# microscopy-processing/FlowDenoising

Hardware: NVIDIA B200
Metric: Mvoxels/s OF-Gaussian denoise (higher is better)
Workload: dtype f32

## Files before the change

### flowdenoising_b200/csrc/flow.cu

```cuda
#include <math.h>
#include <stdlib.h>
#include <string.h>

#include <atomic>

#include "fdn_internal.cuh"

namespace fdn {

struct FlowIterArgs {
    const float* R;
    int64_t R_stride;
    SlotMap map0, map1;
    const float* flow_in;
    float* flow_out;
    int h, w, m;
    int n;
    int LS;
    int strips;
    double scale;
    double* carry;
    unsigned long long* flags;
    unsigned long long epoch;
    unsigned* ctl;
// ... 160 lines not shown
        constexpr bool kStatic = MT > 0 && TR == 2 * MT + 2;
        const bool steady = kStatic && y0 >= TR && y0 + TR - 1 + m <= h - 1 && y0 + m >= 5 && y0 + TR - 1 + m < h - 5;
        if (active && steady) {
            if constexpr (kStatic) {
                constexpr int RRs = 2 * MT + 2;
                double* tq = tile + q;
                float* rg = ring + t;
#pragma unroll
                for (int r = 0; r < TR; r++) {
                    update_matrices_px<false>(R0a, R0b, R1a, R1b, fl[r], xcl, y0 + r + MT, h, w, Mv, colb, sxc);
#pragma unroll
                    for (int c = 0; c < 5; c++) {
                        rg[(((MT + r) % RRs) * 5 + c) * NT] = Mv[c];
                        const float d = __fsub_rn(Mv[c], rg[(((MT + 1 + r) % RRs) * 5 + c) * NT]);
                        vs[c] = __dadd_rn(vs[c], (double)d);
                        tq[(r * 5 + c) * LS] = vs[c];
                    }
                }
                next_row += TR;
            }
        } else if (active) {
            double* tq = tile + q;
#pragma unroll
            for (int r = 0; r < TR; r++) {
                const int y = y0 + r;
                if (y < h) {
                    if (next_row <= min(y + m, h - 1)) {
                        update_matrices_px(R0a, R0b, R1a, R1b, fl[r], xcl, next_row, h, w, Mv);
#pragma unroll
                        for (int c = 0; c < 5; c++) ring_new[c * NT] = Mv[c];
                        ring_new += 5 * NT;
                        if (ring_new >= ring_end) ring_new -= RR * 5 * NT;
                        next_row++;
                    } else {
                        const float* last = (ring_new == ring + t ? ring_end + t : ring_new) - 5 * NT;
#pragma unroll
                        for (int c = 0; c < 5; c++) Mv[c] = last[c * NT];
                    }
#pragma unroll
                    for (int c = 0; c < 5; c++) {
                        const float d = __fsub_rn(Mv[c], ring_old[c * NT]);
                        vs[c] = __dadd_rn(vs[c], (double)d);
                        tq[(r * 5 + c) * LS] = vs[c];
                    }
                    if (y >= m + 1) {
                        ring_old += 5 * NT;
                        if (ring_old >= ring_end) ring_old -= RR * 5 * NT;
                    }
                }
            }
        }
        if (t == 0 && k > 0) {
            const unsigned long long want = a.epoch + (unsigned long long)tile_idx + 1ull;
            while (*flag_in < want) __nanosleep(20);
            __threadfence();
        }
        __syncthreads();
        if (active) {
#pragma unroll
            for (int r = 0; r < TR; r++) {
                const int row = y0 + TR + r + m;
                if (row < h) fl[r] = __ldg(fin + row * w + xcl);
            }
        }
        if (t < 5 * TR) {
            const int r = t / 5, c = t - r * 5;
            const int y = y0 + r;
            if (y < h) {
                double* line = tile + (r * 5 + c) * LS;
                double S;
                if (k == 0) {
                    S = __dmul_rn(line[m + 1], (double)(m + 2));
                    for (int x = 1; x < m; x++) S = __dadd_rn(S, line[m + 1 + x]);
                } else {
                    S = __ldcg(carry_in + (int64_t)y * 5 + c);
                }
                const int off = 2 * m + 1;
                constexpr int HB = 8;
                int i = 0;
                if (ncols >= HB) {
                    double d[HB];
#pragma unroll
                    for (int u = 0; u < HB; u++) d[u] = __dsub_rn(line[u + off], line[u]);
                    for (; i + 2 * HB <= ncols; i += HB) {
                        double d2[HB];
#pragma unroll
                        for (int u = 0; u < HB; u++) d2[u] = __dsub_rn(line[i + HB + u + off], line[i + HB + u]);
#pragma unroll
                        for (int u = 0; u < HB; u++) {
                            S = __dadd_rn(S, d[u]);
                            line[i + u] = S;
                        }
#pragma unroll
                        for (int u = 0; u < HB; u++) d[u] = d2[u];
                    }
#pragma unroll
                    for (int u = 0; u < HB; u++) {
                        S = __dadd_rn(S, d[u]);
                        line[i + u] = S;
                    }
                    i += HB;
                }
                for (; i < ncols; i++) {
                    S = __dadd_rn(S, __dsub_rn(line[i + off], line[i]));
                    line[i] = S;
                }
                if (k + 1 < a.strips) {
                    __stcg(carry_out + (int64_t)y * 5 + c, S);
                    __threadfence();
                }
            }
        }
        __syncthreads();
        if (t == 0 && k + 1 < a.strips) *flag_out = a.epoch + (unsigned long long)tile_idx + 1ull;
        if (core) {
            const double* tt = tile + t;
#pragma unroll
            for (int r = 0; r < TR; r++) {
                const int y = y0 + r;
                if (y < h) {
                    double g[5];
#pragma unroll
                    for (int c = 0; c < 5; c++) g[c] = __dmul_rn(tt[(r * 5 + c) * LS], a.scale);
                    const double det = __dadd_rn(__dsub_rn(__dmul_rn(g[0], g[2]), __dmul_rn(g[1], g[1])), 1e-3);
                    const double idet = __drcp_rn(det);
                    float2 o;
                    o.x = (float)__dmul_rn(__dsub_rn(__dmul_rn(g[0], g[4]), __dmul_rn(g[1], g[3])), idet);
                    o.y = (float)__dmul_rn(__dsub_rn(__dmul_rn(g[2], g[3]), __dmul_rn(g[1], g[4])), idet);
                    fout[y * w + x0 + t] = o;
                }
            }
        }
        __syncthreads();
    }
    if (t == 0) {
        __threadfence();
        if (atomicAdd(a.ctl + 1, 1u) == gridDim.x - 1) { a.ctl[0] = 0; a.ctl[1] = 0; }
    }
}


struct RowIn {
    float2 f;
    float4 c03;
    float c4;
};

template <int MT, int NT_>
struct WsCfg {
    static constexpr int NT = NT_;
    static constexpr int RR = 2 * MT + 2;
    static constexpr int TR = 5 * RR <= 32 ? RR : RR / 2;
    static constexpr int TPP = RR / TR;
#ifndef FDN_WS_SR4
#define FDN_WS_SR4 2
#endif
    static constexpr int SR = MT == 4 ? FDN_WS_SR4 : 3;
    static constexpr int NB = (TR + SR - 1) / SR;
    static constexpr int HALO = 2 * MT + 1;
    static constexpr int CWMAX = (NT - HALO) & ~3;
    static constexpr int NCH = (CWMAX + 31) / 32;
    static constexpr int LS = NT + 2;
#ifndef FDN_WS_NBUF
#define FDN_WS_NBUF 2
#endif
    static constexpr int NBUF = FDN_WS_NBUF;
    static constexpr size_t tiles_bytes = NBUF * sizeof(double) * TR * 5 * LS + 128;
    static constexpr size_t smem_bytes = tiles_bytes + 8 * NBUF * NCH + 16;
    static_assert(5 * TR <= 32, "phase H runs in one warp");
    static_assert(TR * TPP == RR && (TPP == 1 || TPP == 2), "a ring period is one tile or the two shared-memory tiles");
    static_assert(HALO + 8 <= 17, "the scan's register window spans two 8-column sets and one more column");
};

struct Taps {
    float4 p00, p01, p10, p11;
    float q00, q01, q10, q11;
};

template <int PF>
__device__ __forceinline__ Taps ws_gather(const float2 f, const float4* __restrict__ R1a, const float* __restrict__ R1b,
                                          int x, int y, int h, int w)
{
    const int x1 = (int)floorf(__fadd_rn((float)x, f.x)), y1 = (int)floorf(__fadd_rn((float)y, f.y));
    const int yc = min(max(y1, 0), h - 2), xc = min(max(x1, 0), w - 2);
    const int g = yc * w + xc;
    if (PF > 0) {
        const int gp = min(yc + PF + 1, h - 1) * w + xc;
        asm volatile("prefetch.global.L1 [%0];" :: "l"(R1a + gp));
        asm volatile("prefetch.global.L1 [%0];" :: "l"(R1b + gp));
    }
    Taps t;
    t.p00 = __ldg(R1a + g); t.p01 = __ldg(R1a + g + 1); t.p10 = __ldg(R1a + g + w); t.p11 = __ldg(R1a + g + w + 1);
    t.q00 = __ldg(R1b + g); t.q01 = __ldg(R1b + g + 1); t.q10 = __ldg(R1b + g + w); t.q11 = __ldg(R1b + g + w + 1);
    return t;
}

__device__ __forceinline__ void ws_matrices_px(const RowIn& in, const Taps& tp, int x, int y, int h, int w, float sxc,
                                               float M[5])
{
    const float dx = in.f.x, dy = in.f.y;
    float fx = __fadd_rn((float)x, dx), fy = __fadd_rn((float)y, dy);
    const int x1 = (int)floorf(fx), y1 = (int)floorf(fy);
    fx = __fsub_rn(fx, (float)x1);
    fy = __fsub_rn(fy, (float)y1);
    const float4 c03 = in.c03;
    const float c4 = in.c4;
    const bool in_img = (unsigned)x1 < (unsigned)(w - 1) && (unsigned)y1 < (unsigned)(h - 1);
    const float ofx = __fsub_rn(1.f, fx), ofy = __fsub_rn(1.f, fy);
    const float a00 = __fmul_rn(ofx, ofy), a01 = __fmul_rn(fx, ofy), a10 = __fmul_rn(ofx, fy), a11 = __fmul_rn(fx, fy);
#define FDN_BILIN(v00, v01, v10, v11) \
    __fadd_rn(__fadd_rn(__fadd_rn(__fmul_rn(a00, v00), __fmul_rn(a01, v01)), __fmul_rn(a10, v10)), __fmul_rn(a11, v11))
    float r2 = FDN_BILIN(tp.p00.x, tp.p01.x, tp.p10.x, tp.p11.x);
    float r3 = FDN_BILIN(tp.p00.y, tp.p01.y, tp.p10.y, tp.p11.y);
    float r4 = FDN_BILIN(tp.p00.z, tp.p01.z, tp.p10.z, tp.p11.z);
    float r5 = FDN_BILIN(tp.p00.w, tp.p01.w, tp.p10.w, tp.p11.w);
    float r6 = FDN_BILIN(tp.q00, tp.q01, tp.q10, tp.q11);
#undef FDN_BILIN
    r4 = __fmul_rn(__fadd_rn(c03.z, r4), 0.5f);
    r5 = __fmul_rn(__fadd_rn(c03.w, r5), 0.5f);
    r6 = __fmul_rn(__fadd_rn(c4, r6), 0.25f);
    r2 = in_img ? r2 : 0.f;
    r3 = in_img ? r3 : 0.f;
    r4 = in_img ? r4 : c03.z;
    r5 = in_img ? r5 : c03.w;
    r6 = in_img ? r6 : __fmul_rn(c4, 0.5f);
    r2 = __fmul_rn(__fsub_rn(c03.x, r2), 0.5f);
    r3 = __fmul_rn(__fsub_rn(c03.y, r3), 0.5f);
    r2 = __fadd_rn(r2, __fadd_rn(__fmul_rn(r4, dy), __fmul_rn(r6, dx)));
    r3 = __fadd_rn(r3, __fadd_rn(__fmul_rn(r6, dy), __fmul_rn(r5, dx)));
    float s = sxc;
    s = __fmul_rn(s, y < 5 ? (y < 2 ? 0.14f : 0.4472f) : 1.f);
    s = __fmul_rn(s, y >= h - 5 ? (h - y - 1 < 2 ? 0.14f : 0.4472f) : 1.f);
    r2 = __fmul_rn(r2, s); r3 = __fmul_rn(r3, s); r4 = __fmul_rn(r4, s);
    r5 = __fmul_rn(r5, s); r6 = __fmul_rn(r6, s);
    M[0] = __fadd_rn(__fmul_rn(r4, r4), __fmul_rn(r6, r6));
    M[1] = __fmul_rn(__fadd_rn(r4, r5), r6);
    M[2] = __fadd_rn(__fmul_rn(r5, r5), __fmul_rn(r6, r6));
    M[3] = __fadd_rn(__fmul_rn(r4, r2), __fmul_rn(r6, r3));
    M[4] = __fadd_rn(__fmul_rn(r6, r2), __fmul_rn(r5, r3));
}

__device__ __forceinline__ double ws_win(const double2 (&W0)[4], const double2 (&W1)[4], const double2& X, int idx)
{
    return idx < 8 ? ((idx & 1) ? W0[idx >> 1].y : W0[idx >> 1].x)
                   : idx < 16 ? ((idx & 1) ? W1[(idx - 8) >> 1].y : W1[(idx - 8) >> 1].x) : X.x;
}
template <int OFF>
__device__ __forceinline__ void ws_diffs(double (&D)[8], const double2 (&W0)[4], const double2 (&W1)[4], const double2& X)
{
#pragma unroll
    for (int u = 0; u < 8; u++) D[u] = __dsub_rn(ws_win(W0, W1, X, u + OFF), ws_win(W0, W1, X, u));
}

#ifdef FDN_WS_EXPERIMENTS
#define FDN_WS_EXP(bit) (wa.exp & (bit))
#else
#define FDN_WS_EXP(bit) (0)
#endif
#ifndef FDN_WS_HC
#define FDN_WS_HC 8
#endif
#ifndef FDN_WS_PF
#define FDN_WS_PF 6
#endif
#ifndef FDN_WS_L2PF
#define FDN_WS_L2PF 0
#endif
#ifndef FDN_WS_SOLVE_SLEEP
#define FDN_WS_SOLVE_SLEEP 100
#endif
#define FDN_WS_MAX_ITERS 3

struct WsArgs {
    const float* R;
    int64_t R_stride;
    SlotMap map0, map1;
    const float* fin[FDN_WS_MAX_ITERS];
    float* fout[FDN_WS_MAX_ITERS];
    int n, iters;
    int h, w, CW, strips;
    double scale;
    int exp;
    unsigned tag;
    ulonglong2* packets;
    unsigned* ctl;
    unsigned* done;
};

__device__ __forceinline__ void nbar_sync(int id, int count)
{
    asm volatile("bar.sync %0, %1;" :: "r"(id), "r"(count) : "memory");
}
__device__ __forceinline__ void nbar_arrive(int id, int count)
{
    asm volatile("bar.arrive %0, %1;" :: "r"(id), "r"(count) : "memory");
}
__device__ __forceinline__ unsigned ld_acquire_u32(const unsigned* p)
{
    unsigned v;
    asm volatile("ld.acquire.gpu.global.u32 %0, [%1];" : "=r"(v) : "l"(p) : "memory");
    return v;
}

template <int MT, int NT_>
__global__ void __launch_bounds__(NT_ + 128, 2)
k_flow_iter_ws(WsArgs wa)
{
    using C = WsCfg<MT, NT_>;
    constexpr int NT = C::NT, TR = C::TR, SR = C::SR, RR = C::RR, TPP = C::TPP, NB = C::NB, LS = C::LS, NCH = C::NCH, m = MT;
    constexpr int NBUF = C::NBUF, BAR_FULL = 1, BAR_FREE = 1 + NBUF, BAR_SOLVED = 1 + 2 * NBUF;
    constexpr unsigned WARPS = (NT + 128) / 32;
    extern __shared__ __align__(128) unsigned char smem_ws[];
    double* tiles = reinterpret_cast<double*>(smem_ws);
    unsigned long long* chunk_bar = reinterpret_cast<unsigned long long*>(smem_ws + C::tiles_bytes);
    volatile int* sh = reinterpret_cast<volatile int*>(smem_ws + C::tiles_bytes + 8 * NBUF * NCH);
    const int h = wa.h, w = wa.w;
    const int t = threadIdx.x;
    const unsigned per_it = (unsigned)wa.n * (unsigned)wa.strips;
    if (t == 0) {
        const unsigned tk = atomicAdd(wa.ctl, 1u);
        sh[0] = (int)tk;
        const unsigned it0 = tk / per_it;
        if (it0 > 0) {
            const unsigned b0 = (tk - it0 * per_it) / (unsigned)wa.strips;
            const unsigned* dn = wa.done + (size_t)(it0 - 1) * wa.n + b0;
            while (ld_acquire_u32(dn) < (unsigned)wa.strips) __nanosleep(200);
        }
    }
    if (t < NBUF * NCH) mbar_init(smem_u32(chunk_bar + t), 1);
    __syncthreads();
    const unsigned ticket = (unsigned)sh[0];
    const int it = (int)(ticket / per_it);
    const unsigned rem = ticket - (unsigned)it * per_it;
    const int b = (int)(rem / (unsigned)wa.strips);
    const int k = (int)(rem - (unsigned)b * wa.strips);
    const unsigned tag = wa.tag + (unsigned)it;
    const int CW = wa.CW;
    const int x0 = k * CW;
    const int ncols = min(CW, w - x0);
    const int ntiles = (h + TR - 1) / TR;

    auto warp_exit = [&]() {
        __syncwarp();
        unsigned last = 0;
        if ((t & 31) == 0) {
            __threadfence();
            last = atomicAdd(wa.ctl + 1, 1u) == gridDim.x * WARPS - 1u;
        }
        last = __shfl_sync(0xffffffffu, last, 0);
        if (last) {
            for (int i = t & 31; i < wa.iters * wa.n; i += 32) wa.done[i] = 0;
            if ((t & 31) == 0) { wa.ctl[0] = 0; wa.ctl[1] = 0; }
        }
    };

    if (t >= NT) {
#ifndef FDN_WS_RC4
#define FDN_WS_RC4 168
#define FDN_WS_RS4 88
#endif
        if (MT == 4) asm volatile("setmaxnreg.dec.sync.aligned.u32 %0;" :: "n"(FDN_WS_RS4));
        else asm volatile("setmaxnreg.dec.sync.aligned.u32 80;");
        if (t >= NT + 32) {
            constexpr int NS = 96;
            const int sl = t - (NT + 32);
            float2* fout = reinterpret_cast<float2*>(wa.fout[it]) + (int64_t)b * h * w;
            auto solve_px = [&](const double* tt, int r, float2* dst) {
                double g[5];
#pragma unroll
                for (int c = 0; c < 5; c++) g[c] = __dmul_rn(tt[(r * 5 + c) * LS], wa.scale);
                const double det = __dadd_rn(__dsub_rn(__dmul_rn(g[0], g[2]), __dmul_rn(g[1], g[1])), 1e-3);
                const double idet = __drcp_rn(det);
                float2 o;
                o.x = (float)__dmul_rn(__dsub_rn(__dmul_rn(g[0], g[4]), __dmul_rn(g[1], g[3])), idet);
                o.y = (float)__dmul_rn(__dsub_rn(__dmul_rn(g[2], g[3]), __dmul_rn(g[1], g[4])), idet);
                *dst = o;
            };
            const int sw = sl >> 5, sln = sl & 31;
            const int qlast = (ncols - 1) >> 5;
            for (int j = 0; j < ntiles; j++) {
                const int y0 = j * TR;
                const int buf = j % NBUF;
                const uint32_t bars = smem_u32(chunk_bar + buf * NCH);
                const uint32_t parity = (uint32_t)((j / NBUF) & 1);
                for (int q = sw; q <= qlast; q += NS / 32) {
                    mbar_wait_sleep<FDN_WS_SOLVE_SLEEP>(bars + 8 * q, parity);
                    const int col = q * 32 + sln;
                    if (col < ncols && !FDN_WS_EXP(8)) {
                        const double* tt = tiles + buf * TR * 5 * LS + col;
                        float2* dst = fout + (int64_t)y0 * w + x0 + col;
                        if (y0 + TR <= h) {
#pragma unroll
                            for (int r = 0; r < TR; r++) solve_px(tt, r, dst + r * w);
                        } else {
                            for (int r = 0; r < h - y0; r++) solve_px(tt, r, dst + r * w);
                        }
                    }
                }
                mbar_wait_sleep<FDN_WS_SOLVE_SLEEP>(bars + 8 * qlast, parity);
                nbar_arrive(BAR_FREE + buf, NS + NT);
            }
            if (it + 1 < wa.iters) {
                nbar_sync(BAR_SOLVED, NS);
                if (sl == 0) {
                    __threadfence();
                    atomicAdd(wa.done + (size_t)it * wa.n + b, 1u);
                }
            }
            warp_exit();
            return;
        }
        const int lane = t - NT;
        const int r = lane / 5, c = lane - r * 5;
        ulonglong2* pk_out = wa.packets + ((int64_t)b * wa.strips + k) * h * 5;
        const ulonglong2* pk_in = wa.packets + ((int64_t)b * wa.strips + max(k - 1, 0)) * h * 5;
        constexpr int off = 2 * m + 1;
        static_assert(FDN_WS_HC == 8, "the sliding window below is written for 8-column chunks");
        for (int j = 0; j < ntiles; j++) {
            const int y = j * TR + r;
            const int buf = j % NBUF;
            const uint32_t bars = smem_u32(chunk_bar + buf * NCH);
            nbar_sync(BAR_FULL + buf, NT + 32);
            const unsigned hmask = __ballot_sync(0xffffffffu, lane < 5 * TR && y < h);
            if (lane < 5 * TR && y < h) {
                double* line = tiles + (buf * TR * 5 + r * 5 + c) * LS;
                double2* l2 = reinterpret_cast<double2*>(line);
#define FDN_LOADSET(W, kk)                                                        \
    { W[0] = l2[4 * (kk)]; W[1] = l2[4 * (kk) + 1]; W[2] = l2[4 * (kk) + 2]; W[3] = l2[4 * (kk) + 3];   \
      if (off > 7) xx_ = l2[4 * (kk) + 4]; }
#define FDN_CHAIN8(D, kk)                                                          \
    {                                                                              \
        double2 s0, s1, s2, s3;                                                    \
        S = __dadd_rn(S, D[0]); s0.x = S; S = __dadd_rn(S, D[1]); s0.y = S;        \
        S = __dadd_rn(S, D[2]); s1.x = S; S = __dadd_rn(S, D[3]); s1.y = S;        \
        S = __dadd_rn(S, D[4]); s2.x = S; S = __dadd_rn(S, D[5]); s2.y = S;        \
        S = __dadd_rn(S, D[6]); s3.x = S; S = __dadd_rn(S, D[7]); s3.y = S;        \
        l2[4 * (kk)] = s0; l2[4 * (kk) + 1] = s1; l2[4 * (kk) + 2] = s2; l2[4 * (kk) + 3] = s3; \
    }
#define FDN_CHUNK_DONE(kk)                                                         \
    if (((kk) & 3) == 0 && 8 * (kk) < ncols) {                                     \
        __syncwarp(hmask);                                                         \
        if (lane == 0) mbar_arrive(bars + 8 * (((kk) >> 2) - 1));                  \
    }
                const int n8 = ncols >> 3;
                double2 wa_[4], wb_[4], xx_ = make_double2(0., 0.);
                double d[8];
                FDN_LOADSET(wa_, 0);
                FDN_LOADSET(wb_, 1);
                double S;
                if (k == 0) {
                    S = __dmul_rn(line[m + 1], (double)(m + 2));
#pragma unroll
                    for (int x = 1; x < m; x++) S = __dadd_rn(S, line[m + 1 + x]);
                } else if (FDN_WS_EXP(2)) {
                    S = 0.;
                } else {
                    const ulonglong2* src = pk_in + (int64_t)y * 5 + c;
                    ulonglong2 v = __ldcv(src);
                    while ((unsigned)(v.x >> 32) != tag || (unsigned)(v.y >> 32) != tag) {
                        __nanosleep(32);
                        v = __ldcv(src);
                    }
                    S = __hiloint2double((int)(unsigned)v.y, (int)(unsigned)v.x);
                }
                __syncwarp(hmask);
                if (!FDN_WS_EXP(1)) {
                    ws_diffs<off>(d, wa_, wb_, xx_);
                    int kk = 0;
                    while (kk < n8) {
                        FDN_LOADSET(wa_, kk + 2);
                        FDN_CHAIN8(d, kk);
                        ws_diffs<off>(d, wb_, wa_, xx_);
                        ++kk;
                        FDN_CHUNK_DONE(kk);
                        if (kk == n8) break;
                        FDN_LOADSET(wb_, kk + 2);
                        FDN_CHAIN8(d, kk);
                        ws_diffs<off>(d, wa_, wb_, xx_);
                        ++kk;
                        FDN_CHUNK_DONE(kk);
                    }
                    if (ncols & 4) {
                        double2 s0, s1;
                        S = __dadd_rn(S, d[0]); s0.x = S; S = __dadd_rn(S, d[1]); s0.y = S;
                        S = __dadd_rn(S, d[2]); s1.x = S; S = __dadd_rn(S, d[3]); s1.y = S;
                        l2[4 * n8] = s0; l2[4 * n8 + 1] = s1;
                    }
                }
#undef FDN_LOADSET
#undef FDN_CHAIN8
#undef FDN_CHUNK_DONE
                if (k + 1 < wa.strips) {
                    ulonglong2 o;
                    const unsigned long long tg = (unsigned long long)tag << 32;
                    o.x = tg | (unsigned)__double2loint(S);
                    o.y = tg | (unsigned)__double2hiint(S);
                    __stcg(pk_out + (int64_t)y * 5 + c, o);
                }
            }
            __syncwarp();
            if (lane == 0) mbar_arrive(bars + 8 * ((ncols - 1) >> 5));
        }
        warp_exit();
        return;
    }

    if (MT == 4) asm volatile("setmaxnreg.inc.sync.aligned.u32 %0;" :: "n"(FDN_WS_RC4));
    else asm volatile("setmaxnreg.inc.sync.aligned.u32 176;");
    const int xcl = min(max(x0 - m - 1 + t, 0), w - 1);
    const float sxc = __fmul_rn(xcl < 5 ? (xcl < 2 ? 0.14f : 0.4472f) : 1.f,
                                xcl >= w - 5 ? (w - xcl - 1 < 2 ? 0.14f : 0.4472f) : 1.f);

    const float* R0 = wa.R + (int64_t)wa.map0.slot(b) * wa.R_stride;
    const float* R1 = wa.R + (int64_t)wa.map1.slot(b) * wa.R_stride;
    const float4* R0a = reinterpret_cast<const float4*>(R0);
    const float* R0b = R0 + (int64_t)4 * h * w;
    const float4* R1a = reinterpret_cast<const float4*>(R1);
    const float* R1b = R1 + (int64_t)4 * h * w;
    const float2* fin = reinterpret_cast<const float2*>(wa.fin[it]) + (int64_t)b * h * w;

    auto load_row = [&](int y) {
        RowIn in;
        const int idx = min(y, h - 1) * w + xcl;
        asm volatile("ld.global.cg.v2.f32 {%0, %1}, [%2];" : "=f"(in.f.x), "=f"(in.f.y) : "l"(fin + idx));
        asm("ld.global.nc.L1::no_allocate.v4.f32 {%0, %1, %2, %3}, [%4];"
                     : "=f"(in.c03.x), "=f"(in.c03.y), "=f"(in.c03.z), "=f"(in.c03.w) : "l"(R0a + idx));
        asm("ld.global.nc.L1::no_allocate.f32 %0, [%1];" : "=f"(in.c4) : "l"(R0b + idx));
#if FDN_WS_L2PF
        const int idp = min(y + (FDN_WS_L2PF > 0 ? FDN_WS_L2PF : -FDN_WS_L2PF) * TR, h - 1) * w + xcl;
#if FDN_WS_L2PF > 0
        asm volatile("prefetch.global.L2 [%0];" :: "l"(fin + idp));
        asm volatile("prefetch.global.L2 [%0];" :: "l"(R0a + idp));
        asm volatile("prefetch.global.L2 [%0];" :: "l"(R0b + idp));
#else
        asm volatile("prefetch.global.L1 [%0];" :: "l"(fin + idp));
        asm volatile("prefetch.global.L1 [%0];" :: "l"(R0a + idp));
        asm volatile("prefetch.global.L1 [%0];" :: "l"(R0b + idp));
#endif
#endif
        return in;
    };

    float Mring[RR][5];
    double vs[5];
    RowIn cur[TR];
    {
#pragma unroll
        for (int y = 0; y < m; y++) {
            const RowIn in = load_row(y);
            const Taps tp = ws_gather<0>(in.f, R1a, R1b, xcl, min(y, h - 1), h, w);
            ws_matrices_px(in, tp, xcl, min(y, h - 1), h, w, sxc, Mring[y]);
        }
        const float mp2 = (float)(m + 2);
#pragma unroll
        for (int c = 0; c < 5; c++) vs[c] = (double)__fmul_rn(Mring[0][c], mp2);
#pragma unroll
        for (int y = 1; y < m; y++)
#pragma unroll
            for (int c = 0; c < 5; c++) vs[c] = __dadd_rn(vs[c], (double)Mring[y][c]);
#pragma unroll
        for (int s = m; s < RR; s++)
#pragma unroll
            for (int c = 0; c < 5; c++) Mring[s][c] = Mring[0][c];
#pragma unroll
        for (int r = 0; r < TR; r++) cur[r] = load_row(r + m);
    }

    for (int jp = 0; jp < ntiles; jp += TPP) {
#pragma unroll
        for (int tp = 0; tp < TPP; tp++) {
            const int j = jp + tp;
            if (TPP > 1 && j >= ntiles) break;
            const int y0 = j * TR;
            const int buf = (TPP == 2 && NBUF == 2) ? tp : j % NBUF;
            double* tq = tiles + buf * TR * 5 * LS + t;
            if (j >= NBUF) nbar_sync(BAR_FREE + buf, 96 + NT);
#pragma unroll
            for (int blk = 0; blk < NB; blk++) {
                Taps tps[SR];
#pragma unroll
                for (int rr = 0; rr < SR; rr++) {
                    const int r = blk * SR + rr;
                    if (r < TR) tps[rr] = ws_gather<FDN_WS_PF>(cur[r].f, R1a, R1b, xcl, min(y0 + r + m, h - 1), h, w);
                }
                float Mv[SR][5];
#pragma unroll
                for (int rr = 0; rr < SR; rr++) {
                    const int r = blk * SR + rr;
                    if (r < TR) ws_matrices_px(cur[r], tps[rr], xcl, min(y0 + r + m, h - 1), h, w, sxc, Mv[rr]);
                }
                if (wa.tag != 0 && !FDN_WS_EXP(4)) {
#pragma unroll
                    for (int rr = 0; rr < SR; rr++) {
                        const int r = blk * SR + rr;
                        if (r < TR) {
                            const int snew = (tp * TR + r + m) % RR, sold = (tp * TR + r + m + 1) % RR;
#pragma unroll
                            for (int c = 0; c < 5; c++) {
                                const float d = __fsub_rn(Mv[rr][c], Mring[sold][c]);
                                Mring[snew][c] = Mv[rr][c];
                                vs[c] = __dadd_rn(vs[c], (double)d);
                                tq[(r * 5 + c) * LS] = vs[c];
                            }
                        }
                    }
                }
#pragma unroll
                for (int rr = 0; rr < SR; rr++) {
                    const int r = blk * SR + rr;
                    if (r < TR) cur[r] = load_row(y0 + TR + r + m);
                }
            }
#ifndef FDN_WS_NOFENCE
            __threadfence_block();
#endif
            nbar_arrive(BAR_FULL + buf, NT + 32);
        }
    }
    warp_exit();
}

static std::atomic<unsigned long long> g_flow_epoch{1};
static std::atomic<int> g_flow_variant{1};
void set_flow_iter_variant(int v) { g_flow_variant.store(v ? 1 : 0); }

static int strip_width(int w) { return w > 96 ? 128 : 32; }

static unsigned next_packet_tags(int cnt)
{
    for (;;) {
        const unsigned lo = (unsigned)g_flow_epoch.fetch_add((unsigned long long)cnt);
        if (lo != 0 && lo <= 0xffffffffu - (unsigned)cnt) return lo;
    }
}

static int ws_strip_width(int w, int cwmax)
{
    const int strips = (int)cdiv(w, cwmax);
    return (int)((cdiv(w, strips) + 3) / 4 * 4);
}
#define FDN_WS_NT 128
typedef WsCfg<2, FDN_WS_NT> WsCfg2;
typedef WsCfg<4, FDN_WS_NT> WsCfg4;
static int ws_strips_max(int w)
{
    const int a = (int)cdiv(w, ws_strip_width(w, WsCfg2::CWMAX)), b = (int)cdiv(w, ws_strip_width(w, WsCfg4::CWMAX));
    return a > b ? a : b;
}

static size_t align256(size_t v) { return (v + 255) / 256 * 256; }

int flow_scratch_make(void* scratch, size_t bytes, int cap_n, int nlev, const int* hs, const int* ws, FlowScratch* fs)
{
    fs->base = static_cast<char*>(scratch);
    fs->bytes = bytes;
    fs->cap_n = cap_n; fs->H = 0; fs->W = 0;
    fs->flag_strips = 0; fs->packet_rows = 0; fs->carry_rows = 0;
    for (int k = 0; k < nlev; k++) {
        const int h = hs[k], w = ws[k];
        const int strips = (int)cdiv(w, strip_width(w));
        if (h > fs->H) fs->H = h;
        if (w > fs->W) fs->W = w;
        if (strips > fs->flag_strips) fs->flag_strips = strips;
        if ((int64_t)ws_strips_max(w) * h > fs->packet_rows) fs->packet_rows = (int64_t)ws_strips_max(w) * h;
        if ((int64_t)strips * h > fs->carry_rows) fs->carry_rows = (int64_t)strips * h;
    }
    size_t off = 256;
    fs->off_done = off;    off += align256(sizeof(unsigned) * FDN_WS_MAX_ITERS * (size_t)cap_n);
    fs->off_flags = off;   off += align256(sizeof(unsigned long long) * (size_t)cap_n * fs->flag_strips);
    fs->off_packets = off; off += align256(sizeof(ulonglong2) * 5 * (size_t)cap_n * (size_t)fs->packet_rows);
    fs->off_carry = off;   off += align256(sizeof(double) * 5 * (size_t)cap_n * (size_t)fs->carry_rows);
    if (scratch && bytes < off) {
        set_error("flow iteration scratch too small: need %zu bytes, got %zu", off, bytes);
        return FDN_ERR_WORKSPACE;
    }
    fs->bytes = off;
    return FDN_OK;
}

size_t flow_iter_scratch_bytes(int cap_n, int nlev, const int* hs, const int* ws)
{
    FlowScratch fs;
    flow_scratch_make(nullptr, 0, cap_n, nlev, hs, ws, &fs);
    return fs.bytes;
}

int flow_iter_scratch_init(const FlowScratch& fs, cudaStream_t st)
{
    FDN_CUDA(cudaMemsetAsync(fs.base, 0, fs.bytes, st));
    return FDN_OK;
}

static bool first_use_on_device(std::atomic<bool> (&seen)[64])
{
    int dev = 0;
    if (cudaGetDevice(&dev) != cudaSuccess || dev < 0 || dev >= 64) return true;
    return !seen[dev].exchange(true);
}

template <int CW, int TR, int MT, int MINB>
static int launch_flow_variant(const FlowIterArgs& a, unsigned blocks, size_t smem, cudaStream_t st)
{
    static std::atomic<bool> seen[64];
    if (first_use_on_device(seen))
        FDN_CUDA(cudaFuncSetAttribute(k_flow_iter<CW, TR, MT, MINB>, cudaFuncAttributeMaxDynamicSharedMemorySize,
                                      200 * 1024));
    k_flow_iter<CW, TR, MT, MINB><<<blocks, CW + 32, smem, st>>>(a);
    return FDN_OK;
}

static int launch_flow_iter_strip(const float* R, int64_t R_stride, SlotMap map0, SlotMap map1, const float* flow_in,
                                  float* flow_out, int n, int h, int w, int winsize, const FlowScratch& fs,
                                  cudaStream_t st)
{
    FlowIterArgs a;
    a.R = R; a.R_stride = R_stride;
    a.h = h; a.w = w; a.m = winsize / 2;
    a.n = n;
    a.scale = 1. / ((double)winsize * winsize);
    const int m = a.m;
    const int RR = 2 * m + 2;
    const bool wide = w > 96;
    const int CW = strip_width(w);
    const int NT = CW + 32;
    const int TR = (wide && m == 2) ? 6 : 4;
    a.strips = (int)cdiv(w, CW);
    a.LS = tile_line_stride(CW, m);
    FDN_CHECK_ARG(a.strips <= fs.flag_strips && (int64_t)a.strips * h <= fs.carry_rows,
                  "flow iteration scratch was not sized for a %d x %d level", h, w);
    FDN_CHECK_ARG((int64_t)n * a.strips < (1ll << 31), "too many image pairs in one launch");
    a.ctl = reinterpret_cast<unsigned*>(fs.base);
    a.flags = reinterpret_cast<unsigned long long*>(fs.base + fs.off_flags);
    a.carry = reinterpret_cast<double*>(fs.base + fs.off_carry);
    const size_t smem = sizeof(double) * TR * 5 * a.LS + sizeof(float) * RR * 5 * NT;
    const unsigned long long tiles = (unsigned long long)cdiv(h, TR);
    a.map0 = map0; a.map1 = map1;
    a.flow_in = flow_in; a.flow_out = flow_out;
    a.epoch = g_flow_epoch.fetch_add(tiles + 1);
    ProfScope ps(K_FLOW_ITER, 56.0 * n * h * w, st, n, h, w);
    const unsigned blocks = (unsigned)a.strips * (unsigned)n;
    int rc;
    if (wide) {
        if (m == 2) rc = launch_flow_variant<128, 6, 2, 4>(a, blocks, smem, st);
        else if (m == 4) rc = launch_flow_variant<128, 4, 4, 4>(a, blocks, smem, st);
        else rc = launch_flow_variant<128, 4, 0, 4>(a, blocks, smem, st);
    } else {
        if (m == 2) rc = launch_flow_variant<32, 4, 2, 8>(a, blocks, smem, st);
        else rc = launch_flow_variant<32, 4, 0, 8>(a, blocks, smem, st);
    }
    if (rc) return rc;
    FDN_LAUNCHED("k_flow_iter");
    return FDN_OK;
}

template <int MT>
static int launch_ws(const WsArgs& wa, unsigned blocks, cudaStream_t st)
{
    using C = WsCfg<MT, FDN_WS_NT>;
    static std::atomic<bool> seen[64];
    if (first_use_on_device(seen)) {
        FDN_CUDA(cudaFuncSetAttribute(k_flow_iter_ws<MT, FDN_WS_NT>, cudaFuncAttributeMaxDynamicSharedMemorySize,
                                      (int)C::smem_bytes));
        FDN_CUDA(cudaFuncSetAttribute(k_flow_iter_ws<MT, FDN_WS_NT>, cudaFuncAttributePreferredSharedMemoryCarveout,
                                      (int)((2 * (C::smem_bytes + 1024) * 100 + 228 * 1024 - 1) / (228 * 1024))));
        if (getenv("FDN_DEBUG")) {
            int nb = 0;
            cudaOccupancyMaxActiveBlocksPerMultiprocessor(&nb, k_flow_iter_ws<MT, FDN_WS_NT>, FDN_WS_NT + 128, C::smem_bytes);
            fprintf(stderr, "[fdn] k_flow_iter_ws<%d>: %d blocks/SM, %zu B shared memory per block\n", MT, nb,
                    (size_t)C::smem_bytes);
        }
    }
    k_flow_iter_ws<MT, FDN_WS_NT><<<blocks, FDN_WS_NT + 128, C::smem_bytes, st>>>(wa);
    return FDN_OK;
}

int launch_flow_level(const float* R, int64_t R_stride, SlotMap map0, SlotMap map1, float* cur, float* bufa, float* bufb,
                      int n, int h, int w, int winsize, int iters, const FlowScratch& fs, cudaStream_t st,
                      float** result)
{
    FDN_CHECK_ARG(winsize >= 1 && winsize <= 31, "winsize %d unsupported (1..31)", winsize);
    FDN_CHECK_ARG(cur != bufa && cur != bufb && bufa != bufb, "the three flow buffers must be distinct");
    FDN_CHECK_ARG((int64_t)h * w < (1ll << 28), "level image too large");
    FDN_CHECK_ARG(n >= 1 && n <= fs.cap_n && h <= fs.H && w <= fs.W, "flow iteration scratch was sized for %d pairs of %d x %d",
                  fs.cap_n, fs.H, fs.W);
    float* bufs[3] = {cur, bufa, bufb};
    const int m = winsize / 2;
    const bool win = g_flow_variant.load() == 1 && (m == 2 || m == 4) && w % 4 == 0 && w >= 64 && h >= 16 &&
                     (reinterpret_cast<uintptr_t>(R) & 15) == 0 && R_stride % 4 == 0;
    if (!win) {
        for (int i = 0; i < iters; i++) {
            int rc = launch_flow_iter_strip(R, R_stride, map0, map1, bufs[i % 3], bufs[(i + 1) % 3], n, h, w, winsize, fs,
                                            st);
            if (rc) return rc;
        }
        *result = bufs[iters % 3];
        return FDN_OK;
    }
    WsArgs wa;
    wa.R = R; wa.R_stride = R_stride;
    wa.map0 = map0; wa.map1 = map1;
    wa.n = n; wa.h = h; wa.w = w;
    wa.scale = 1. / ((double)winsize * winsize);
    wa.CW = ws_strip_width(w, m == 2 ? WsCfg2::CWMAX : WsCfg4::CWMAX);
    wa.strips = (int)cdiv(w, wa.CW);
    FDN_CHECK_ARG((int64_t)wa.strips * h <= fs.packet_rows, "flow iteration scratch was not sized for a %d x %d level",
                  h, w);
    FDN_CHECK_ARG((int64_t)n * wa.strips * FDN_WS_MAX_ITERS < (1ll << 31), "too many image pairs in one launch");
    wa.ctl = reinterpret_cast<unsigned*>(fs.base);
    wa.done = reinterpret_cast<unsigned*>(fs.base + fs.off_done);
    wa.packets = reinterpret_cast<ulonglong2*>(fs.base + fs.off_packets);
    wa.exp = 0;
#ifdef FDN_WS_EXPERIMENTS
    { const char* e = getenv("FDN_EXP"); wa.exp = e ? atoi(e) : 0; }
#endif
#ifdef FDN_WS_ITERS_PER_LAUNCH
    const int per_launch = FDN_WS_ITERS_PER_LAUNCH;
#else
    const int per_launch = FDN_WS_MAX_ITERS;
#endif
    for (int i0 = 0; i0 < iters; i0 += per_launch) {
        const int cnt = iters - i0 < per_launch ? iters - i0 : per_launch;
        for (int i = 0; i < cnt; i++) {
            wa.fin[i] = bufs[(i0 + i) % 3];
            wa.fout[i] = bufs[(i0 + i + 1) % 3];
        }
        for (int i = cnt; i < FDN_WS_MAX_ITERS; i++) { wa.fin[i] = nullptr; wa.fout[i] = nullptr; }
        wa.iters = cnt;
        wa.tag = next_packet_tags(cnt);
        ProfScope ps(K_FLOW_ITER, 56.0 * cnt * n * h * w, st, n, h, w);
        const unsigned blocks = (unsigned)cnt * (unsigned)n * (unsigned)wa.strips;
        int rc = m == 2 ? launch_ws<2>(wa, blocks, st) : launch_ws<4>(wa, blocks, st);
        if (rc) return rc;
        FDN_LAUNCHED("k_flow_iter_ws");
    }
    *result = bufs[iters % 3];
    return FDN_OK;
}

#define GW_NT 128
#define GW_TR 8
#define GW_MAX_M 15

struct GaussIterArgs {
    const float* R;
    int64_t R_stride;
    SlotMap map0, map1;
    const float* flow_in;
    float* flow_out;
    int h, w, m;
    int CW, strips;
    float k[GW_MAX_M + 1];
};

static void gauss_window_taps(int m, float* k)
{
    const double sigma = m * 0.3;
    double s = 1;
    k[0] = (float)s;
    for (int i = 1; i <= m; i++) {
        const float t = (float)exp(-i * i / (2 * sigma * sigma));
        k[i] = t;
        s += t * 2;
    }
    s = 1. / s;
    for (int i = 0; i <= m; i++) k[i] = (float)(k[i] * s);
}

template <int MT>
__global__ void __launch_bounds__(GW_NT, 4)
k_flow_gauss_iter(GaussIterArgs a)
{
    constexpr bool kReg = MT > 0;
    extern __shared__ __align__(16) float gw_smem[];
    const int m = kReg ? MT : a.m;
    const int RR = 2 * m + 1;
    const int TR = kReg ? 2 * MT + 1 : GW_TR;
    const int h = a.h, w = a.w;
    float* tile = gw_smem;
    float* ring = gw_smem + TR * 5 * GW_NT + threadIdx.x;

    const int t = threadIdx.x;
    const int b = blockIdx.x / a.strips, k = blockIdx.x - b * a.strips;
    const int x0 = k * a.CW;
    const int xcol = x0 - m + t;
    const bool active = xcol <= w - 1 + m;
    const int xcl = min(max(xcol, 0), w - 1);
    const bool core = t < a.CW && x0 + t < w;

    const float* R0 = a.R + (int64_t)a.map0.slot(b) * a.R_stride;
    const float* R1 = a.R + (int64_t)a.map1.slot(b) * a.R_stride;
    const float4* R0a = reinterpret_cast<const float4*>(R0);
    const float4* R1a = reinterpret_cast<const float4*>(R1);
    const float* R0b = R0 + (int64_t)4 * h * w;
    const float* R1b = R1 + (int64_t)4 * h * w;
    const float2* fin = reinterpret_cast<const float2*>(a.flow_in) + (int64_t)b * h * w;
    float2* fout = reinterpret_cast<float2*>(a.flow_out) + (int64_t)b * h * w;

    auto matrices = [&](int row, float M[5]) {
        update_matrices_px(R0a, R0b, R1a, R1b, __ldg(fin + row * w + xcl), xcl, row, h, w, M);
    };
    auto solve_row = [&](int r, int y) {
        const float* tl = tile + r * 5 * GW_NT + t + m;
        double g[5];
#pragma unroll
        for (int c = 0; c < 5; c++) {
            const float* v = tl + c * GW_NT;
            float s = __fmul_rn(v[0], a.k[0]);
            if (kReg) {
#pragma unroll
                for (int i = 1; i <= MT; i++) s = __fadd_rn(s, __fmul_rn(__fadd_rn(v[i], v[-i]), a.k[i]));
            } else {
                for (int i = 1; i <= m; i++) s = __fadd_rn(s, __fmul_rn(__fadd_rn(v[i], v[-i]), a.k[i]));
            }
            g[c] = (double)s;
        }
        const double det = __dadd_rn(__dsub_rn(__dmul_rn(g[0], g[2]), __dmul_rn(g[1], g[1])), 1e-3);
        const double idet = __drcp_rn(det);
        float2 o;
        o.x = (float)__dmul_rn(__dsub_rn(__dmul_rn(g[0], g[4]), __dmul_rn(g[1], g[3])), idet);
        o.y = (float)__dmul_rn(__dsub_rn(__dmul_rn(g[2], g[3]), __dmul_rn(g[1], g[4])), idet);
        fout[y * w + x0 + t] = o;
    };

    if constexpr (kReg) {
        constexpr int RRc = 2 * MT + 1;
        float rg[RRc][5];
        if (active) {
            float M0[5];
            matrices(0, M0);
#pragma unroll
            for (int j = -MT; j <= 0; j++)
#pragma unroll
                for (int c = 0; c < 5; c++) rg[(j + RRc) % RRc][c] = M0[c];
#pragma unroll
            for (int j = 1; j < MT; j++) matrices(min(j, h - 1), rg[j]);
        }
        for (int y0 = 0; y0 < h; y0 += RRc) {
            if (active) {
#pragma unroll
                for (int r = 0; r < RRc; r++) {
                    const int y = y0 + r;
                    if (y < h) {
                        matrices(min(y + MT, h - 1), rg[(r + MT) % RRc]);
#pragma unroll
                        for (int c = 0; c < 5; c++) {
                            float s = __fmul_rn(rg[r][c], a.k[0]);
#pragma unroll
                            for (int i = 1; i <= MT; i++)
                                s = __fadd_rn(s, __fmul_rn(__fadd_rn(rg[(r + i) % RRc][c], rg[(r - i + RRc) % RRc][c]),
                                                          a.k[i]));
                            tile[(r * 5 + c) * GW_NT + t] = s;
                        }
                    }
                }
            }
            __syncthreads();
            if (core) {
#pragma unroll
                for (int r = 0; r < RRc; r++)
                    if (y0 + r < h) solve_row(r, y0 + r);
            }
            __syncthreads();
        }
    } else {
        if (active) {
            float M0[5];
            matrices(0, M0);
            for (int j = -m; j <= 0; j++)
#pragma unroll
                for (int c = 0; c < 5; c++) ring[((j + m) * 5 + c) * GW_NT] = M0[c];
            for (int j = 1; j < m; j++) {
                float Mv[5];
                matrices(min(j, h - 1), Mv);
#pragma unroll
                for (int c = 0; c < 5; c++) ring[((j + m) * 5 + c) * GW_NT] = Mv[c];
            }
        }
        int sy = m;
        for (int y0 = 0; y0 < h; y0 += GW_TR) {
            if (active) {
                for (int r = 0; r < GW_TR && y0 + r < h; r++) {
                    const int y = y0 + r;
                    int sn = sy + m;
// ... 373 lines not shown
```

Measured before the change: 245.3.

## Run two independent strip pipelines per block with one scan and one solve warp each

Each block now holds two pipelines, each with 128 compute threads, and a shared producer warpgroup. That group has one scan warp and one solve warp per pipeline, replacing the old layout of one scan warp and three solve warps. Each pipeline takes its own ticket, named barriers and tile region, and the wait on the previous iteration moves from block start to each pipeline's compute group, so the two tickets do not block each other. Launch bounds become one block per SM with a higher compute register budget, and the mt=4 scan row count goes from 2 to 3. The aim is denser per-SM scheduling and less overhead per block. The cost is fewer solver threads per pipeline, which could become a bottleneck, plus an odd tail ticket that leaves one pipeline idle.

```diff
diff --git a/flowdenoising_b200/csrc/flow.cu b/flowdenoising_b200/csrc/flow.cu
--- a/flowdenoising_b200/csrc/flow.cu
+++ b/flowdenoising_b200/csrc/flow.cu
@@ -336,10 +336,13 @@
     static constexpr int RR = 2 * MT + 2;
     static constexpr int TR = 5 * RR <= 32 ? RR : RR / 2;
     static constexpr int TPP = RR / TR;
+#ifndef FDN_WS_SR2
+#define FDN_WS_SR2 3
+#endif
 #ifndef FDN_WS_SR4
-#define FDN_WS_SR4 2
+#define FDN_WS_SR4 3
 #endif
-    static constexpr int SR = MT == 4 ? FDN_WS_SR4 : 3;
+    static constexpr int SR = MT == 4 ? FDN_WS_SR4 : FDN_WS_SR2;
     static constexpr int NB = (TR + SR - 1) / SR;
     static constexpr int HALO = 2 * MT + 1;
     static constexpr int CWMAX = (NT - HALO) & ~3;
@@ -349,8 +352,10 @@
 #define FDN_WS_NBUF 2
 #endif
     static constexpr int NBUF = FDN_WS_NBUF;
+    static constexpr int NP = 2;
     static constexpr size_t tiles_bytes = NBUF * sizeof(double) * TR * 5 * LS + 128;
-    static constexpr size_t smem_bytes = tiles_bytes + 8 * NBUF * NCH + 16;
+    static constexpr size_t smem_bytes = NP * tiles_bytes + 8 * NP * NBUF * NCH + 16;
+    static_assert(tiles_bytes % 16 == 0, "the tiles of the second pipeline must stay 16-byte aligned");
     static_assert(5 * TR <= 32, "phase H runs in one warp");
     static_assert(TR * TPP == RR && (TPP == 1 || TPP == 2), "a ring period is one tile or the two shared-memory tiles");
     static_assert(HALO + 8 <= 17, "the scan's register window spans two 8-column sets and one more column");
@@ -471,6 +476,13 @@
     unsigned* done;
 };
 
+template <typename T>
+__device__ __forceinline__ T ws_pick(T const (&p)[FDN_WS_MAX_ITERS], int i)
+{
+    static_assert(FDN_WS_MAX_ITERS == 3, "one select per iteration of a launch");
+    return i == 0 ? p[0] : i == 1 ? p[1] : p[2];
+}
+
 __device__ __forceinline__ void nbar_sync(int id, int count)
 {
     asm volatile("bar.sync %0, %1;" :: "r"(id), "r"(count) : "memory");
@@ -486,34 +498,52 @@
     return v;
 }
 
+#ifndef FDN_WS_RC
+#define FDN_WS_RC 208
+#endif
+#ifndef FDN_WS_RS
+#define FDN_WS_RS 88
+#endif
 template <int MT, int NT_>
-__global__ void __launch_bounds__(NT_ + 128, 2)
+__global__ void __launch_bounds__(2 * NT_ + 128, 1)
 k_flow_iter_ws(WsArgs wa)
 {
     using C = WsCfg<MT, NT_>;
     constexpr int NT = C::NT, TR = C::TR, SR = C::SR, RR = C::RR, TPP = C::TPP, NB = C::NB, LS = C::LS, NCH = C::NCH, m = MT;
-    constexpr int NBUF = C::NBUF, BAR_FULL = 1, BAR_FREE = 1 + NBUF, BAR_SOLVED = 1 + 2 * NBUF;
-    constexpr unsigned WARPS = (NT + 128) / 32;
+    constexpr int NBUF = C::NBUF, NP = C::NP;
+    constexpr unsigned WARPS = (NP * NT + 128) / 32;
+    static_assert(NP == 2 && NT == 128, "warpgroup 2 holds one scan warp and one solve warp per pipeline");
+    static_assert(1 + NP * (2 * NBUF + 1) <= 16, "named barriers of the pipelines");
     extern __shared__ __align__(128) unsigned char smem_ws[];
-    double* tiles = reinterpret_cast<double*>(smem_ws);
-    unsigned long long* chunk_bar = reinterpret_cast<unsigned long long*>(smem_ws + C::tiles_bytes);
-    volatile int* sh = reinterpret_cast<volatile int*>(smem_ws + C::tiles_bytes + 8 * NBUF * NCH);
+    const int t = threadIdx.x;
+    const int p = t < NP * NT ? t / NT : ((t - NP * NT) >> 5) & 1;
+    unsigned long long* chunk_bars = reinterpret_cast<unsigned long long*>(smem_ws + NP * C::tiles_bytes);
+    double* tiles = reinterpret_cast<double*>(smem_ws + p * C::tiles_bytes);
+    unsigned long long* chunk_bar = chunk_bars + p * NBUF * NCH;
+    volatile int* sh = reinterpret_cast<volatile int*>(chunk_bars + NP * NBUF * NCH);
+    const int BAR_FULL = 1 + p * (2 * NBUF + 1), BAR_FREE = BAR_FULL + NBUF, BAR_START = BAR_FULL + 2 * NBUF;
     const int h = wa.h, w = wa.w;
-    const int t = threadIdx.x;
     const unsigned per_it = (unsigned)wa.n * (unsigned)wa.strips;
-    if (t == 0) {
-        const unsigned tk = atomicAdd(wa.ctl, 1u);
-        sh[0] = (int)tk;
-        const unsigned it0 = tk / per_it;
-        if (it0 > 0) {
-            const unsigned b0 = (tk - it0 * per_it) / (unsigned)wa.strips;
-            const unsigned* dn = wa.done + (size_t)(it0 - 1) * wa.n + b0;
-            while (ld_acquire_u32(dn) < (unsigned)wa.strips) __nanosleep(200);
-        }
-    }
-    if (t < NBUF * NCH) mbar_init(smem_u32(chunk_bar + t), 1);
+    if (t < NP * NT && t % NT == 0) sh[p] = (int)atomicAdd(wa.ctl, 1u);
+    if (t < NP * NBUF * NCH) mbar_init(smem_u32(chunk_bars + t), 1);
     __syncthreads();
-    const unsigned ticket = (unsigned)sh[0];
+
+    auto warp_exit = [&]() {
+        __syncwarp();
+        unsigned last = 0;
+        if ((t & 31) == 0) {
+            __threadfence();
+            last = atomicAdd(wa.ctl + 1, 1u) == gridDim.x * WARPS - 1u;
+        }
+        last = __shfl_sync(0xffffffffu, last, 0);
+        if (last) {
+            for (int i = t & 31; i < wa.iters * wa.n; i += 32) wa.done[i] = 0;
+            if ((t & 31) == 0) { wa.ctl[0] = 0; wa.ctl[1] = 0; }
+        }
+    };
+
+    const unsigned ticket = (unsigned)sh[p];
+    const bool idle = ticket >= (unsigned)wa.iters * per_it;
     const int it = (int)(ticket / per_it);
     const unsigned rem = ticket - (unsigned)it * per_it;
     const int b = (int)(rem / (unsigned)wa.strips);
@@ -524,31 +554,16 @@
     const int ncols = min(CW, w - x0);
     const int ntiles = (h + TR - 1) / TR;
 
-    auto warp_exit = [&]() {
-        __syncwarp();
-        unsigned last = 0;
-        if ((t & 31) == 0) {
-            __threadfence();
-            last = atomicAdd(wa.ctl + 1, 1u) == gridDim.x * WARPS - 1u;
-        }
-        last = __shfl_sync(0xffffffffu, last, 0);
-        if (last) {
-            for (int i = t & 31; i < wa.iters * wa.n; i += 32) wa.done[i] = 0;
-            if ((t & 31) == 0) { wa.ctl[0] = 0; wa.ctl[1] = 0; }
-        }
-    };
-
-    if (t >= NT) {
-#ifndef FDN_WS_RC4
-#define FDN_WS_RC4 168
-#define FDN_WS_RS4 88
-#endif
-        if (MT == 4) asm volatile("setmaxnreg.dec.sync.aligned.u32 %0;" :: "n"(FDN_WS_RS4));
-        else asm volatile("setmaxnreg.dec.sync.aligned.u32 80;");
-        if (t >= NT + 32) {
-            constexpr int NS = 96;
-            const int sl = t - (NT + 32);
-            float2* fout = reinterpret_cast<float2*>(wa.fout[it]) + (int64_t)b * h * w;
+    if (t >= NP * NT) {
+        asm volatile("setmaxnreg.dec.sync.aligned.u32 %0;" :: "n"(FDN_WS_RS));
+        if (idle) {
+            warp_exit();
+            return;
+        }
+        if (t >= NP * NT + 64) {
+            constexpr int NS = 32;
+            const int sln = t & 31;
+            float2* fout = reinterpret_cast<float2*>(ws_pick(wa.fout, it)) + (int64_t)b * h * w;
             auto solve_px = [&](const double* tt, int r, float2* dst) {
                 double g[5];
 #pragma unroll
@@ -560,14 +575,13 @@
                 o.y = (float)__dmul_rn(__dsub_rn(__dmul_rn(g[2], g[3]), __dmul_rn(g[1], g[4])), idet);
                 *dst = o;
             };
-            const int sw = sl >> 5, sln = sl & 31;
             const int qlast = (ncols - 1) >> 5;
             for (int j = 0; j < ntiles; j++) {
                 const int y0 = j * TR;
                 const int buf = j % NBUF;
                 const uint32_t bars = smem_u32(chunk_bar + buf * NCH);
                 const uint32_t parity = (uint32_t)((j / NBUF) & 1);
-                for (int q = sw; q <= qlast; q += NS / 32) {
+                for (int q = 0; q <= qlast; q++) {
                     mbar_wait_sleep<FDN_WS_SOLVE_SLEEP>(bars + 8 * q, parity);
                     const int col = q * 32 + sln;
                     if (col < ncols && !FDN_WS_EXP(8)) {
@@ -581,12 +595,11 @@
                         }
                     }
                 }
-                mbar_wait_sleep<FDN_WS_SOLVE_SLEEP>(bars + 8 * qlast, parity);
                 nbar_arrive(BAR_FREE + buf, NS + NT);
             }
             if (it + 1 < wa.iters) {
-                nbar_sync(BAR_SOLVED, NS);
-                if (sl == 0) {
+                __syncwarp();
+                if (sln == 0) {
                     __threadfence();
                     atomicAdd(wa.done + (size_t)it * wa.n + b, 1u);
                 }
@@ -594,7 +607,7 @@
             warp_exit();
             return;
         }
-        const int lane = t - NT;
+        const int lane = t & 31;
         const int r = lane / 5, c = lane - r * 5;
         ulonglong2* pk_out = wa.packets + ((int64_t)b * wa.strips + k) * h * 5;
         const ulonglong2* pk_in = wa.packets + ((int64_t)b * wa.strips + max(k - 1, 0)) * h * 5;
@@ -689,9 +702,20 @@
         return;
     }
 
-    if (MT == 4) asm volatile("setmaxnreg.inc.sync.aligned.u32 %0;" :: "n"(FDN_WS_RC4));
-    else asm volatile("setmaxnreg.inc.sync.aligned.u32 176;");
-    const int xcl = min(max(x0 - m - 1 + t, 0), w - 1);
+    if (idle) {
+        warp_exit();
+        return;
+    }
+    asm volatile("setmaxnreg.inc.sync.aligned.u32 %0;" :: "n"(FDN_WS_RC));
+    if (it > 0) {
+        if (t % NT == 0) {
+            const unsigned* dn = wa.done + (size_t)(it - 1) * wa.n + b;
+            while (ld_acquire_u32(dn) < (unsigned)wa.strips) __nanosleep(200);
+        }
+        nbar_sync(BAR_START, NT);
+    }
+    const int tc = t - p * NT;
+    const int xcl = min(max(x0 - m - 1 + tc, 0), w - 1);
     const float sxc = __fmul_rn(xcl < 5 ? (xcl < 2 ? 0.14f : 0.4472f) : 1.f,
                                 xcl >= w - 5 ? (w - xcl - 1 < 2 ? 0.14f : 0.4472f) : 1.f);
 
@@ -701,7 +725,7 @@
     const float* R0b = R0 + (int64_t)4 * h * w;
     const float4* R1a = reinterpret_cast<const float4*>(R1);
     const float* R1b = R1 + (int64_t)4 * h * w;
-    const float2* fin = reinterpret_cast<const float2*>(wa.fin[it]) + (int64_t)b * h * w;
+    const float2* fin = reinterpret_cast<const float2*>(ws_pick(wa.fin, it)) + (int64_t)b * h * w;
 
     auto load_row = [&](int y) {
         RowIn in;
@@ -757,8 +781,8 @@
             if (TPP > 1 && j >= ntiles) break;
             const int y0 = j * TR;
             const int buf = (TPP == 2 && NBUF == 2) ? tp : j % NBUF;
-            double* tq = tiles + buf * TR * 5 * LS + t;
-            if (j >= NBUF) nbar_sync(BAR_FREE + buf, 96 + NT);
+            double* tq = tiles + buf * TR * 5 * LS + tc;
+            if (j >= NBUF) nbar_sync(BAR_FREE + buf, 32 + NT);
 #pragma unroll
             for (int blk = 0; blk < NB; blk++) {
                 Taps tps[SR];
@@ -946,15 +970,16 @@
         FDN_CUDA(cudaFuncSetAttribute(k_flow_iter_ws<MT, FDN_WS_NT>, cudaFuncAttributeMaxDynamicSharedMemorySize,
                                       (int)C::smem_bytes));
         FDN_CUDA(cudaFuncSetAttribute(k_flow_iter_ws<MT, FDN_WS_NT>, cudaFuncAttributePreferredSharedMemoryCarveout,
-                                      (int)((2 * (C::smem_bytes + 1024) * 100 + 228 * 1024 - 1) / (228 * 1024))));
+                                      (int)(((C::smem_bytes + 1024) * 100 + 228 * 1024 - 1) / (228 * 1024))));
         if (getenv("FDN_DEBUG")) {
             int nb = 0;
-            cudaOccupancyMaxActiveBlocksPerMultiprocessor(&nb, k_flow_iter_ws<MT, FDN_WS_NT>, FDN_WS_NT + 128, C::smem_bytes);
-            fprintf(stderr, "[fdn] k_flow_iter_ws<%d>: %d blocks/SM, %zu B shared memory per block\n", MT, nb,
-                    (size_t)C::smem_bytes);
-        }
-    }
-    k_flow_iter_ws<MT, FDN_WS_NT><<<blocks, FDN_WS_NT + 128, C::smem_bytes, st>>>(wa);
+            cudaOccupancyMaxActiveBlocksPerMultiprocessor(&nb, k_flow_iter_ws<MT, FDN_WS_NT>, C::NP * FDN_WS_NT + 128,
+                                                          C::smem_bytes);
+            fprintf(stderr, "[fdn] k_flow_iter_ws<%d>: %d blocks/SM of %d threads, %zu B shared memory per block\n", MT,
+                    nb, C::NP * FDN_WS_NT + 128, (size_t)C::smem_bytes);
+        }
+    }
+    k_flow_iter_ws<MT, FDN_WS_NT><<<blocks, C::NP * FDN_WS_NT + 128, C::smem_bytes, st>>>(wa);
     return FDN_OK;
 }
 
@@ -1012,7 +1037,7 @@
         wa.iters = cnt;
         wa.tag = next_packet_tags(cnt);
         ProfScope ps(K_FLOW_ITER, 56.0 * cnt * n * h * w, st, n, h, w);
-        const unsigned blocks = (unsigned)cnt * (unsigned)n * (unsigned)wa.strips;
+        const unsigned blocks = (unsigned)cdiv((int64_t)cnt * n * wa.strips, WsCfg2::NP);
         int rc = m == 2 ? launch_ws<2>(wa, blocks, st) : launch_ws<4>(wa, blocks, st);
         if (rc) return rc;
         FDN_LAUNCHED("k_flow_iter_ws");
```

New measurement: 232.4 (median of 6 runs). -5.2%, worse.
